# Iselix/kwiiyatta

Hardware: AMD Instinct MI355X
Metric: frames/sec end-to-end analyse->align->convert->synth, 48 kHz 5 ms hop (higher is better)
Workload: dtype f64; 1 GPU; config3: 48 kHz source (10 s, T=2001) + target (11 s, T=2201) pairs: CheapTrick+D4C of both, pad with freshly drawn silent spectra, sp2mc, FastDTW(radius 32) align, GMM(64 comp, D=144)+MLPG convert, mc2sp, WORLD synthesis; pairs_per_gpu=32, streams_per_gpu=4, GPU_MAX_HW_QUEUES=4, launch=the whole step is one captured HIP graph, gmm_model_prepared=once per converter (the per-mixture matrices depend on the GMM only), parallelism=pairs in lockstep x32 per GPU, pair-per-GPU x1, no collective

## Files before the change

### kwiiyatta_amd/csrc/kwy_d4c.hip

```cpp
#include <math.h>

#include <vector>

#include "kwy_internal.hpp"

#define D4C_SAFE 0.000000000001
#define D4C_FLOOR_F0 47.0
#define D4C_FREQ_INTERVAL 3000.0
#define D4C_UPPER_LIMIT 15000.0
#define D4C_MAX_BANDS 8

enum { D4C_HANNING = 1, D4C_BLACKMAN = 2 };

__device__ __forceinline__ double d4c_window(int type, int i, int half, double ratio, int fs, double cf0) {
  const double c1 = kwy_cos_pi_range(KWY_PI * ((2.0 * (i - half) / ratio) / fs) * cf0);
  return type == D4C_HANNING ? 0.5 * c1 + 0.5 : 0.42 + 0.5 * c1 + 0.08 * (2.0 * c1 * c1 - 1.0);
}

struct d4c_window_walk {
  double c, s, cd, sd;
  __device__ __forceinline__ d4c_window_walk(int i0, int step, int half, double ratio, int fs, double cf0) {
    kwy_sincos_pi_range(KWY_PI * ((2.0 * (i0 - half) / ratio) / fs) * cf0, &s, &c);
    sincos(KWY_PI * ((2.0 * step / ratio) / fs) * cf0, &sd, &cd);
  }
// ... 554 lines not shown
    constexpr int Q = (H / 2) / NT;
    static_assert(RK == 2 * Q + 1, "pairs per thread");
#pragma unroll
    for (int q = 0; q < Q; ++q)
      kwy_rfft_pair_power2_w<LOG2N - 1>(B, tid + NT * q, kwy_tw_hex(d4c_opaque(twb), HEX * q), &pv[2 * q], &pv[2 * q + 1]);
    pv[2 * Q] = 0.0;
    if (tid == 0) {
      double pm;
      kwy_rfft_pair_power2_w<LOG2N - 1>(B, H / 2, kwy_c{0.0, -1.0}, &pv[2 * Q], &pm);
    }
    __syncthreads();
#pragma unroll
    for (int q = 0; q < Q; ++q) {
      const int k = tid + NT * q;
      P[k] = pv[2 * q];
      P[H - k] = pv[2 * q + 1];
    }
    if (tid == 0) P[H / 2] = pv[2 * Q];
  }
  __syncthreads();
  d4c_dc_correction<NT>(P, S, cf0, p.fs, N);
  d4c_linear_smoothing_regs<NT, RK>(P, pv, S, tot, cf0, p.fs, N);

  D4C_STAMP(9);
#pragma unroll
  for (int r = 0; r < RP; ++r) {
    const int pp = DRAIN ? kwy_drain_bin<LOG2N - 1>(r, tid) : tid + NT * r;
    if (pp < H / 2) { Dv[pp] = cen_lo[r]; Dv[H - pp] = cen_hi[r]; }
  }
  if (tid == 0) Dv[H / 2] = mid[2];
  __syncthreads();
  d4c_dc_correction<NT>(Dv, S, cf0, p.fs, N);
#pragma unroll
  for (int r = 0; r < RK; ++r)
    if (tid + NT * r <= H) Dv[tid + NT * r] = Dv[tid + NT * r] / pv[r];
  __syncthreads();
  const int kdv = p.dv_len - 1;
  d4c_linear_smoothing<NT>(Dv, Dv, S, tot, cf0 / 2.0, p.fs, N, kdv + 2 * ((int)(cf0 * N / p.fs) + 1) + 4);
  d4c_subtract_smoothed<NT>(Dv, S, tot, cf0, p.fs, N, kdv);

  D4C_STAMP(10);
  {
    double *dv = dvbuf + (size_t)frame * p.dv_stride;
    for (int k = tid; k < p.dv_len; k += NT) dv[k] = Dv[k];
  }
  D4C_STAMP(15);
#undef D4C_STAMP
#undef D4C_BODY_TW4
}

template <int LOG2N>
static constexpr size_t d4c_bands_lds() {
  constexpr int N = 1 << LOG2N, H = N / 2, NT = d4c_nt<LOG2N>::value;
  return sizeof(double) * (16 + D4C_MAX_BANDS + 2 + 2 * NT) + sizeof(double) * ((2 * H + 2) + 2) +
         ((sizeof(uint32_t) * KWY_SELECT_WORDS(NT) > sizeof(double) * (2 * H + 4))
              ? sizeof(uint32_t) * KWY_SELECT_WORDS(NT) - sizeof(double) * (2 * H + 4) : 0);
}

template <int LOG2N, bool SPARSE>
__global__ __launch_bounds__(d4c_nt<LOG2N>::value, LOG2N >= 13 ? 2 : 4) void k_d4c_bands(
    d4c_batch batch, d4c_params p, const kwy_c *__restrict__ twH, const kwy_c *__restrict__ twP,
    const kwy_c *__restrict__ twN, const double *__restrict__ nuttall, long long *__restrict__ dbg) {
  constexpr int N = 1 << LOG2N, H = N / 2;
  constexpr int NT = d4c_nt<LOG2N>::value;
  constexpr int E = N / NT;
  constexpr int RK = (H + 1 + NT - 1) / NT;
  constexpr int HEX = 16 * NT / N;
  constexpr bool DRAIN = d4c_drain<LOG2N>::value;
#define D4C_STAMP(n) do { if (dbg && threadIdx.x == 0 && blockIdx.x == (unsigned)dbg[63]) dbg[n] = clock64(); } while (0)
  extern __shared__ double smem[];
  double *red = smem;
  double *coarse = red + 16;
  double *wns = coarse + D4C_MAX_BANDS + 2;
  kwy_c *B = (kwy_c *)(wns + 2 * NT);
  double *Bd = (double *)B;
  uint32_t *hist = (uint32_t *)B;

  const int tid = threadIdx.x;
  const int utt = batch.find(blockIdx.x);
  const int64_t frame = (int)blockIdx.x - batch.start[utt];
  const double *__restrict__ dvbuf = batch.u[utt].dvbuf;
  double *__restrict__ out = batch.u[utt].out;
  const double f0v = kwy_uniform(batch.u[utt].f0[frame]);
  if (f0v == 0.0 || kwy_uniform(batch.u[utt].ap0[frame]) <= p.threshold) return;
  const double cf0 = kwy_uniform(f0v > D4C_FLOOR_F0 ? f0v : D4C_FLOOR_F0);
  const double *Dv = dvbuf + (size_t)frame * p.dv_stride;
  D4C_STAMP(16);

  const int boundary = __builtin_amdgcn_readfirstlane(kwy_matlab_round(N * 8.0 / p.window_length));
  const int half_window_length = p.window_length / 2;
  constexpr bool sparse = SPARSE;
  double ns0 = 0.0, ns1 = 0.0, ns2 = 0.0, nutr[4] = {0.0, 0.0, 0.0, 0.0};
  if constexpr (sparse) {
    if (2 * tid < p.window_length) ns0 = nuttall[2 * tid];
    if (2 * tid + 1 < p.window_length) ns1 = nuttall[2 * tid + 1];
    wns[2 * tid] = ns0; wns[2 * tid + 1] = ns1;
  } else {
#pragma unroll
    for (int r = 0; r < 4; ++r)
      if (tid + NT * r < p.window_length) nutr[r] = nuttall[tid + NT * r];
  }
  const bool mine0 = sparse && tid < H / 8 && 2 * tid < p.window_length;
  const bool mine1 = sparse && tid < H / 8 && 2 * tid + 1 < p.window_length;
  const double *Dfirst = Dv + ((int)(D4C_FREQ_INTERVAL * N / p.fs) - half_window_length);
  double nx0 = (mine0 && p.nbands > 0) ? Dfirst[2 * tid] : 0.0;
  double nx1 = (mine1 && p.nbands > 0) ? Dfirst[2 * tid + 1] : 0.0;
  for (int b = 0; b < p.nbands; ++b) {
    const int tid = kwy_tid_opaque();
    kwy_c tw4[4];
    kwy_fft_thread_twiddles<LOG2N - 1, NT>(twH + (tid - (int)threadIdx.x), tw4);
    const kwy_c twb = twN[tid];
    const double *Dc = Dv + ((int)(D4C_FREQ_INTERVAL * (b + 1) * N / p.fs) - half_window_length);
    const double c0 = nx0, c1 = nx1;
    if (b == 1) D4C_STAMP(17);
    {
      const double *Dn = Dv + ((int)(D4C_FREQ_INTERVAL * (b + 2) * N / p.fs) - half_window_length);
      const bool more = b + 1 < p.nbands;
      nx0 = (mine0 && more) ? Dn[2 * tid] : 0.0;
      nx1 = (mine1 && more) ? Dn[2 * tid + 1] : 0.0;
    }
    if constexpr (sparse) {
      kwy_c a0 = {c0 * wns[2 * tid], c1 * wns[2 * tid + 1]}, a1 = {0.0, 0.0};
      if (tid == 0 && 2 * (H / 8) < p.window_length) a1.x = Dc[2 * (H / 8)] * nuttall[2 * (H / 8)];
      kwy_fft_pass8_first_sparse_core<LOG2N - 1, NT, false>(B, kwy_tw_reg{tw4[0]}, a0, a1);
      kwy_fft_inplace_rest_w<LOG2N - 1, NT, false, !DRAIN>(B, tw4, twP);
      if (b == 1) D4C_STAMP(18);
    } else {
#pragma unroll
      for (int r = 0; r < E; ++r) {
        const int j = tid + NT * r;
        Bd[j] = (r < 4 && j < p.window_length) ? Dc[j] * nutr[r < 4 ? r : 0] : 0.0;
      }
      __syncthreads();
      kwy_fft_inplace_w<LOG2N - 1, NT, false, !DRAIN>(B, tw4, twP);
    }
    unsigned long long key[RK];
    constexpr int Q = (H / 2) / NT;
    static_assert(RK == 2 * Q + 1, "pairs per thread");
    if constexpr (DRAIN) {
      static_assert(Q == 4 && sizeof(uint32_t) * KWY_SELECT_WORDS(NT) <= sizeof(kwy_c) * NT, "exchange clear of the histogram");
      kwy_c lo[4], hi[4], md;
      kwy_fft_tail4_drain<LOG2N - 1, NT, false>(B, lo, hi, md);
      const kwy_c twc = D4C_DRAIN_TWC(twN, NT, tid);
      double pw[8];
#pragma unroll
      for (int s = 0; s < 4; ++s) {
        if (s == 0 && tid == 0) kwy_rfft_pair_power2_dc(lo[0], &pw[0], &pw[1]);
        else kwy_rfft_pair_power2_v(lo[s], hi[s], kwy_drain_tw<LOG2N - 1, NT>(s, d4c_opaque(twb), twc), &pw[2 * s], &pw[2 * s + 1]);
      }
      key[2 * Q] = ~0ull;
      if (tid == 0) {
        double pk, pm;
        kwy_rfft_pair_power2_v(md, md, kwy_c{0.0, -1.0}, &pk, &pm);
        key[2 * Q] = (unsigned long long)__double_as_longlong(pk);
      } else {
        B[2 * NT - tid] = kwy_c{pw[4], pw[5]};
        B[4 * NT - tid] = kwy_c{pw[6], pw[7]};
      }
      __syncthreads();
      if (tid != 0) {
        const kwy_c v1 = B[NT + tid], v3 = B[3 * NT + tid];
        pw[4] = v1.x; pw[5] = v1.y; pw[6] = v3.x; pw[7] = v3.y;
      }
      key[0] = (unsigned long long)__double_as_longlong(pw[0]); key[1] = (unsigned long long)__double_as_longlong(pw[1]);
      key[2] = (unsigned long long)__double_as_longlong(pw[4]); key[3] = (unsigned long long)__double_as_longlong(pw[5]);
      key[4] = (unsigned long long)__double_as_longlong(pw[2]); key[5] = (unsigned long long)__double_as_longlong(pw[3]);
      key[6] = (unsigned long long)__double_as_longlong(pw[6]); key[7] = (unsigned long long)__double_as_longlong(pw[7]);
    } else {
#pragma unroll
      for (int q = 0; q < Q; ++q) {
        double pk, pm;
        kwy_rfft_pair_power2_w<LOG2N - 1>(B, tid + NT * q, kwy_tw_hex(d4c_opaque(twb), HEX * q), &pk, &pm);
        key[2 * q] = (unsigned long long)__double_as_longlong(pk);
        key[2 * q + 1] = (unsigned long long)__double_as_longlong(pm);
      }
      key[2 * Q] = ~0ull;
      if (tid == 0) {
        double pk, pm;
        kwy_rfft_pair_power2_w<LOG2N - 1>(B, H / 2, kwy_c{0.0, -1.0}, &pk, &pm);
        key[2 * Q] = (unsigned long long)__double_as_longlong(pk);
      }
      __syncthreads();
    }
    if (b == 1) D4C_STAMP(19);
    double nsmall, nall;
    kwy_block_smallest_sum<RK, NT>(key, H + 1, H - boundary, hist, red, &nsmall, &nall);
    if (b == 1) D4C_STAMP(20);
    if (dbg && tid == 0 && blockIdx.x == (unsigned)dbg[63])
      for (int q = 0; q < 12; ++q) dbg[24 + 12 * (b & 1) + q] = hist[2 * KWY_SELECT_BINS + q];
    if (tid == 0) {
      double cv = 10 * log10(nsmall / nall);
      cv = cv + (cf0 - 100) / 50.0;
      coarse[b + 1] = cv < 0.0 ? cv : 0.0;
    }
    __syncthreads();
  }
  D4C_STAMP(21);
  if (tid == 0) {
    coarse[0] = -60.0;
    coarse[p.nbands + 1] = -D4C_SAFE;
  }
  __syncthreads();
  double *o = out + frame * p.K;
  const int nn = p.nbands + 2;
  for (int k = tid; k < p.K; k += NT) {
    double xi = (double)k * p.fs / p.fft_size;
    int seg = min((int)(xi / D4C_FREQ_INTERVAL) + 1, p.nbands + 1);
    if (seg < 1) seg = 1;
    if (seg > nn - 1) seg = nn - 1;
    double xa = (seg - 1 <= p.nbands) ? (seg - 1) * D4C_FREQ_INTERVAL : p.fs / 2.0;
    double xb = (seg <= p.nbands) ? seg * D4C_FREQ_INTERVAL : p.fs / 2.0;
    double sfrac = (xi - xa) / (xb - xa);
    double v = coarse[seg - 1] + sfrac * (coarse[seg] - coarse[seg - 1]);
    o[k] = exp10(v / 20.0);
  }
  D4C_STAMP(22);
#undef D4C_STAMP
}

template <int LOG2N>
static int launch_lt(kwy_ctx *ctx, const d4c_batch &b, int fs) {
  constexpr int N = 1 << LOG2N, H = N / 2;
  const kwy_c *twH, *twN, *twP;
  const uint4 *poly;
  KWY_TRY(kwy_get_twiddles(ctx, LOG2N - 1, &twH));
  KWY_TRY(kwy_get_twiddle_powers(ctx, LOG2N - 1, &twP));
  KWY_TRY(kwy_get_twiddles(ctx, LOG2N, &twN));
  constexpr int NT = d4c_nt<LOG2N>::value;
  KWY_TRY(kwy_get_poly_multi(ctx, N / NT, NT, &poly));
  size_t lds = sizeof(kwy_c) * (H + 1) + sizeof(double) * 8 + sizeof(uint32_t) * KWY_EBASE_WORDS;
  KWY_HIP(hipFuncSetAttribute((const void *)k_d4c_lovetrain<LOG2N, NT>,
                              hipFuncAttributeMaxDynamicSharedMemorySize, (int)lds));
  KWY_PROF(ctx, "k_d4c_lovetrain", hipLaunchKernelGGL((k_d4c_lovetrain<LOG2N, NT>), dim3((unsigned)b.start[b.n]), dim3(NT), lds,
                     ctx->stream, b, fs, kwy_randn(ctx), poly, twH, twP, twN));
  KWY_HIP(hipGetLastError());
  return KWY_OK;
}

template <int LOG2N>
static int launch_body(kwy_ctx *ctx, const d4c_batch &b, const d4c_params &p, const double *nuttall) {
  constexpr int N = 1 << LOG2N, H = N / 2;
  const kwy_c *twH, *twN, *twP;
  const uint4 *poly;
  KWY_TRY(kwy_get_twiddles(ctx, LOG2N - 1, &twH));
  KWY_TRY(kwy_get_twiddle_powers(ctx, LOG2N - 1, &twP));
  KWY_TRY(kwy_get_twiddles(ctx, LOG2N, &twN));
  constexpr int NT = d4c_nt<LOG2N>::value;
  KWY_TRY(kwy_get_poly_multi(ctx, N / NT, NT, &poly));
// ... 198 lines not shown
```

### kwiiyatta_amd/csrc/kwy_device.hpp

```cpp
#pragma once

#include <hip/hip_runtime.h>
#include <stdint.h>

#define KWY_THREADS 256
#define KWY_WAVES (KWY_THREADS / 64)
#define KWY_PI 3.1415926535897932384

struct kwy_rng {
  uint32_t x, y, z, w;
};

__device__ __forceinline__ void kwy_rng_seed(kwy_rng &r) {
  r.x = 123456789u; r.y = 362436069u; r.z = 521288629u; r.w = 88675123u;
}

__device__ __forceinline__ uint32_t kwy_rng_step(kwy_rng &r) {
  uint32_t t = r.x ^ (r.x << 11);
  r.x = r.y; r.y = r.z; r.z = r.w;
  r.w = (r.w ^ (r.w >> 19)) ^ (t ^ (t >> 8));
  return r.w;
}

__device__ __forceinline__ uint32_t kwy_rng_randn_raw(kwy_rng &r) {
// ... 373 lines not shown
}

template <int NT, class F>
__device__ inline void kwy_block_count_scan(F count, int64_t n, uint64_t *__restrict__ offsets, uint64_t *tot) {
  const int t = threadIdx.x;
  const int64_t chunk = (n + NT - 1) / NT;
  const int64_t b0 = t * chunk, b1 = min(n, b0 + chunk);
  uint64_t run = 0;
  for (int64_t i = b0; i < b1; ++i) run += count(i);
  tot[t] = run;
  __syncthreads();
  if (t < 64) {
    constexpr int PER = NT / 64;
    uint64_t a[PER], acc = 0;
#pragma unroll
    for (int q = 0; q < PER; ++q) { a[q] = acc; acc += tot[PER * t + q]; }
    uint64_t inc = acc;
#pragma unroll
    for (int o = 1; o < 64; o <<= 1) {
      const uint64_t up = __shfl_up(inc, o);
      if (t >= o) inc += up;
    }
    const uint64_t excl = inc - acc;
#pragma unroll
    for (int q = 0; q < PER; ++q) tot[PER * t + q] = excl + a[q];
  }
  __syncthreads();
  run = tot[t];
  for (int64_t i = b0; i < b1; ++i) { offsets[i] = run; run += count(i); }
  if (b0 < n && b1 == n) offsets[n] = run;
  if (n == 0 && t == 0) offsets[0] = 0;
}

template <int NT = KWY_THREADS>
__device__ __forceinline__ void kwy_block_sum2(double a, double b, double *red, double *ta, double *tb) {
  a = kwy_wave_sum(a);
  b = kwy_wave_sum(b);
  __syncthreads();
  if ((threadIdx.x & 63) == 0) { red[threadIdx.x >> 6] = a; red[NT / 64 + (threadIdx.x >> 6)] = b; }
  __syncthreads();
  double sa = red[0], sb = red[NT / 64];
#pragma unroll
  for (int i = 1; i < NT / 64; ++i) { sa += red[i]; sb += red[NT / 64 + i]; }
  *ta = sa; *tb = sb;
}

#ifndef KWY_SELECT_BITS
#define KWY_SELECT_BITS 8
#endif
#define KWY_SELECT_BINS (1 << KWY_SELECT_BITS)
#ifndef KWY_SELECT_AGG
#define KWY_SELECT_AGG 0
#endif
#define KWY_SELECT_WORDS(NT) (2 * KWY_SELECT_BINS + 32)
#define KWY_SELECT_LIST (KWY_SELECT_BINS / 2 - 4)

__device__ __forceinline__ uint32_t kwy_wave_max_u32(uint32_t v) {
  v = max(v, (uint32_t)__builtin_amdgcn_update_dpp((int)v, (int)v, 0x101, 0xf, 0xf, false));
  v = max(v, (uint32_t)__builtin_amdgcn_update_dpp((int)v, (int)v, 0x102, 0xf, 0xf, false));
  v = max(v, (uint32_t)__builtin_amdgcn_update_dpp((int)v, (int)v, 0x104, 0xf, 0xf, false));
  v = max(v, (uint32_t)__builtin_amdgcn_update_dpp((int)v, (int)v, 0x108, 0xf, 0xf, false));
  return max(max((uint32_t)__builtin_amdgcn_readlane((int)v, 0), (uint32_t)__builtin_amdgcn_readlane((int)v, 16)),
             max((uint32_t)__builtin_amdgcn_readlane((int)v, 32), (uint32_t)__builtin_amdgcn_readlane((int)v, 48)));
}

__device__ __forceinline__ void kwy_select_scan(const uint32_t *h, int kk, uint32_t *ctl, int lane) {
  constexpr int PERLANE = KWY_SELECT_BINS / 64;
  static_assert(PERLANE % 4 == 0 && PERLANE >= 4, "bins per lane must be a multiple of 4");
  const uint4 *hp = (const uint4 *)h + lane * (PERLANE / 4);
  uint32_t tot = 0;
#pragma unroll
  for (int q = 0; q < PERLANE / 4; ++q) {
    const uint4 c4 = hp[q];
    tot += (c4.x + c4.y) + (c4.z + c4.w);
  }
  uint32_t before = kwy_wave_scan_u32(tot) - tot;
  if ((uint32_t)kk > before && (uint32_t)kk <= before + tot) {
    const uint32_t *hb = h + PERLANE * lane;
    for (int q = 0; q < PERLANE; ++q) {
      const uint32_t c = hb[q];
      if ((uint32_t)kk <= before + c) {
        ctl[0] = PERLANE * lane + q;
        ctl[1] = (uint32_t)kk - before;
        ctl[2] = c;
        ctl[3] = before;
        break;
      }
      before += c;
    }
  }
}

template <bool DESCENDING>
__device__ __forceinline__ void kwy_select_rank(const unsigned long long *list, int pop, int rank, int tid,
                                                unsigned long long *out_key, uint32_t *out_count) {
  if (tid < pop) {
    const unsigned long long mine = list[tid];
    int front = 0, tie_front = 0, ties = 0;
    for (int j = 0; j < pop; j += 4) {
      const ulonglong2 o01 = *(const ulonglong2 *)(list + j), o23 = *(const ulonglong2 *)(list + j + 2);
      const unsigned long long o[4] = {o01.x, o01.y, o23.x, o23.y};
#pragma unroll
      for (int q = 0; q < 4; ++q) {
        const bool in = j + q < pop;
        front += in & (DESCENDING ? o[q] > mine : o[q] < mine);
        const bool eq = in & (o[q] == mine);
        ties += eq;
        tie_front += eq & (j + q < tid);
      }
    }
    if (front + tie_front == rank - 1) { *out_key = mine; out_count[0] = (uint32_t)front; out_count[1] = (uint32_t)ties; }
  }
}

template <int RMAX, int NT = KWY_THREADS>
__device__ inline void kwy_block_smallest_sum(unsigned long long (&key)[RMAX], int n, int m,
                                              uint32_t *hist, double *red, double *sum_small,
                                              double *sum_all) {
  constexpr int BITS = KWY_SELECT_BITS, BINS = 1 << BITS;
  constexpr int TOP_SHIFT = 18;
  const int tid = threadIdx.x, lane = tid & 63, wv = tid >> 6;
  uint32_t *ctlb = hist + 2 * BINS;
  unsigned long long *k64 = (unsigned long long *)(ctlb + 8);
  unsigned long long *list = (unsigned long long *)(hist + BINS);
  unsigned long long vkey;
  int copies;

  uint32_t hmax = 0;
#pragma unroll
  for (int r = 0; r < RMAX; ++r)
    if (tid + NT * r < n) hmax = max(hmax, (uint32_t)(key[r] >> 32));
  hmax = kwy_wave_max_u32(hmax);
  if (lane == 0) ctlb[16 + wv] = hmax;
  for (int i = tid; i < BINS; i += NT) hist[i] = 0;
  if (tid == 0) ctlb[10] = 0;
  __syncthreads();
  hmax = ctlb[16];
#pragma unroll
  for (int i = 1; i < NT / 64; ++i) hmax = max(hmax, ctlb[16 + i]);
  uint32_t dg[RMAX];
#pragma unroll
  for (int r = 0; r < RMAX; ++r) {
    dg[r] = BINS;
    if (NT * r + (tid & ~63) >= n) continue;
    if (tid + NT * r < n) {
      dg[r] = min((hmax - (uint32_t)(key[r] >> 32)) >> TOP_SHIFT, (uint32_t)(BINS - 1));
      atomicAdd(&hist[dg[r]], 1u);
    }
  }
  __syncthreads();
  if (wv == 0) kwy_select_scan(hist, n - m + 1, ctlb, lane);
  __syncthreads();
  const uint32_t chosen = ctlb[0], pop = ctlb[2];
  if (chosen < (uint32_t)(BINS - 1) && pop <= (uint32_t)KWY_SELECT_LIST) {
    const int rank = (int)ctlb[1], above = (int)ctlb[3];
#pragma unroll
    for (int r = 0; r < RMAX; ++r)
      if (dg[r] == chosen) list[atomicAdd(&ctlb[10], 1u)] = key[r];
    __syncthreads();
    kwy_select_rank<true>(list, (int)pop, rank, tid, k64, &ctlb[11]);
    __syncthreads();
    vkey = *k64;
    copies = m - (n - above - (int)ctlb[11] - (int)ctlb[12]);
  } else {
    double lo = INFINITY, hi = 0.0;
#pragma unroll
    for (int r = 0; r < RMAX; ++r) {
      if (tid + NT * r < n) {
        const double x = __longlong_as_double((long long)key[r]);
        lo = fmin(lo, x); hi = fmax(hi, x);
      }
    }
    lo = kwy_wave_min_f64(lo);
    hi = kwy_wave_max_f64(hi);
    if (lane == 0) { red[wv] = lo; red[NT / 64 + wv] = hi; }
    for (int i = tid; i < BINS; i += NT) hist[i] = 0;
    if (tid == 0) ctlb[10] = 0;
    __syncthreads();
    lo = red[0]; hi = red[NT / 64];
#pragma unroll
    for (int i = 1; i < NT / 64; ++i) { lo = fmin(lo, red[i]); hi = fmax(hi, red[NT / 64 + i]); }
    const unsigned long long kmin = (unsigned long long)__double_as_longlong(lo);
    const unsigned long long range = (unsigned long long)__double_as_longlong(hi) - kmin;
    const int top0 = range ? 64 - __clzll((long long)range) : 0;
    const int rounds = (top0 + BITS - 1) / BITS;
#pragma unroll
    for (int r = 0; r < RMAX; ++r) key[r] -= kmin;
    unsigned long long prefix = 0ull;
    int kk = m;
    bool alive[RMAX];
#pragma unroll
    for (int r = 0; r < RMAX; ++r) alive[r] = tid + NT * r < n;
    for (int round = 0; round < rounds; ++round) {
      const int top = top0 - BITS * round;
      const int shift = top - BITS > 0 ? top - BITS : 0;
      const unsigned long long mask = (1ull << (top - shift)) - 1ull;
      uint32_t *h = hist + (round & 1) * BINS, *hn = hist + ((round + 1) & 1) * BINS;
      uint32_t *ctl = ctlb + (round & 1) * 4;
      for (int i = tid; i < BINS; i += NT) hn[i] = 0;
#pragma unroll
      for (int r = 0; r < RMAX; ++r) {
        if (NT * r + (tid & ~63) >= n) continue;
        const int d = (int)((key[r] >> shift) & mask);
#if KWY_SELECT_AGG
        const unsigned long long mm = __ballot(alive[r]);
        if (mm != 0ull) {
          const int leader = __builtin_amdgcn_readfirstlane(__ffsll((long long)mm) - 1);
          const int d0 = __builtin_amdgcn_readlane(d, leader);
          const bool same = alive[r] && d == d0;
          const unsigned long long ms = __ballot(same);
          if (lane == leader) atomicAdd(&h[d0], (uint32_t)__popcll(ms));
          if (alive[r] && !same) atomicAdd(&h[d], 1u);
        }
#else
        if (alive[r]) atomicAdd(&h[d], 1u);
#endif
      }
      __syncthreads();
      if (wv == 0) kwy_select_scan(h, kk, ctl, lane);
      __syncthreads();
      const int chosen_d = (int)ctl[0];
      prefix |= (unsigned long long)chosen_d << shift;
      kk = (int)ctl[1];
#pragma unroll
      for (int r = 0; r < RMAX; ++r) alive[r] = alive[r] && (int)((key[r] >> shift) & mask) == chosen_d;
      const uint32_t left = ctl[2];
      if (left == 1u && round < rounds - 1) {
#pragma unroll
        for (int r = 0; r < RMAX; ++r)
          if (alive[r]) *k64 = key[r];
        __syncthreads();
        prefix = *k64;
        kk = 1;
        break;
      }
      if (left <= (uint32_t)KWY_SELECT_LIST && round < rounds - 1) {
        unsigned long long *lst = (unsigned long long *)hn;
#pragma unroll
        for (int r = 0; r < RMAX; ++r)
          if (alive[r]) lst[atomicAdd(&ctlb[10], 1u)] = key[r];
        __syncthreads();
        kwy_select_rank<false>(lst, (int)left, kk, tid, k64, &ctlb[11]);
        __syncthreads();
        prefix = *k64;
        kk -= (int)ctlb[11];
        break;
      }
    }
    vkey = prefix + kmin;
    copies = kk;
#pragma unroll
    for (int r = 0; r < RMAX; ++r) key[r] += kmin;
  }
  const double vstar = __longlong_as_double((long long)vkey);
  double s_less = 0.0, s_all = 0.0;
#pragma unroll
  for (int r = 0; r < RMAX; ++r) {
    if (tid + NT * r < n) {
      const double x = __longlong_as_double((long long)key[r]);
      s_all += x;
      if (key[r] < vkey) s_less += x;
    }
  }
  double t_less, t_all;
  kwy_block_sum2<NT>(s_less, s_all, red, &t_less, &t_all);
  *sum_small = t_less + (double)copies * vstar;
  *sum_all = t_all;
}

struct __attribute__((aligned(16))) kwy_c { double x, y; };

__device__ __forceinline__ kwy_c cadd(kwy_c a, kwy_c b) { return {a.x + b.x, a.y + b.y}; }
__device__ __forceinline__ kwy_c csub(kwy_c a, kwy_c b) { return {a.x - b.x, a.y - b.y}; }
__device__ __forceinline__ kwy_c cmul(kwy_c a, kwy_c b) {
  return {a.x * b.x - a.y * b.y, a.x * b.y + a.y * b.x};
}
__device__ __forceinline__ kwy_c cmulf(kwy_c a, kwy_c b) {
  return {__builtin_fma(a.x, b.x, -(a.y * b.y)), __builtin_fma(a.x, b.y, a.y * b.x)};
}

__device__ __forceinline__ kwy_c kwy_tw_octant(kwy_c b, int r) {
  const double h = 0.70710678118654752440;
  switch (r & 7) {
    case 0: return b;
    case 1: return {h * (b.x + b.y), h * (b.y - b.x)};
    case 2: return {b.y, -b.x};
    case 3: return {h * (b.y - b.x), h * (-b.x - b.y)};
    case 4: return {-b.x, -b.y};
    case 5: return {h * (-b.x - b.y), h * (b.x - b.y)};
    case 6: return {-b.y, b.x};
    default: return {h * (b.x - b.y), h * (b.x + b.y)};
  }
}

template <bool INV>
__device__ __forceinline__ kwy_c kwy_rot90(kwy_c a) {
  return INV ? kwy_c{-a.y, a.x} : kwy_c{a.y, -a.x};
}

template <bool INV>
__device__ __forceinline__ void kwy_dft8(kwy_c (&a)[8]) {
  const double h = 0.70710678118654752440;
  kwy_c t0 = cadd(a[0], a[4]), t1 = csub(a[0], a[4]);
  kwy_c t2 = cadd(a[2], a[6]), t3 = kwy_rot90<INV>(csub(a[2], a[6]));
  kwy_c t4 = cadd(a[1], a[5]), t5 = csub(a[1], a[5]);
  kwy_c t6 = cadd(a[3], a[7]), t7 = csub(a[3], a[7]);
  kwy_c u0 = cadd(t0, t2), u1 = csub(t0, t2), u2 = cadd(t4, t6), u3 = kwy_rot90<INV>(csub(t4, t6));
  kwy_c c1 = INV ? kwy_c{h * (t5.x - t5.y), h * (t5.x + t5.y)} : kwy_c{h * (t5.x + t5.y), h * (t5.y - t5.x)};
  kwy_c c3 = INV ? kwy_c{h * (-t7.x - t7.y), h * (t7.x - t7.y)} : kwy_c{h * (t7.y - t7.x), h * (-t7.x - t7.y)};
  kwy_c v0 = cadd(t1, t3), v1 = csub(t1, t3), v2 = cadd(c1, c3), v3 = kwy_rot90<INV>(csub(c1, c3));
  a[0] = cadd(u0, u2); a[4] = csub(u0, u2); a[2] = cadd(u1, u3); a[6] = csub(u1, u3);
  a[1] = cadd(v0, v2); a[5] = csub(v0, v2); a[3] = cadd(v1, v3); a[7] = csub(v1, v3);
}

struct kwy_tw_table {
  const kwy_c *tw;
  __device__ __forceinline__ kwy_c operator()(int ps) const { return tw[ps]; }
};
#define KWY_TWP_ENTRY 8
#define KWY_TWP_ENTRIES(LOG2H) ((1 << (LOG2H)) / 512)
// ... 388 lines not shown
```

### kwiiyatta_amd/csrc/kwy_selftest.h

```cpp
#ifndef KWY_SELFTEST_H_
#define KWY_SELFTEST_H_
#ifdef __cplusplus
extern "C" {
#endif
int kwy_debug_smallest_sum_dev(void *stream, const double *values, int problems, int n, int m, double *out);
int kwy_debug_devmath_dev(void *stream, const double *x, int n, double *log_out, double *sin_out, double *cos_out);
int kwy_debug_rfft_paths_dev(void *stream, const double *x, int problems, int log2n, double *out_old, double *out_new);
int kwy_debug_fft_powers_dev(void *stream, const double *x, int problems, int log2h, int nt, int inverse,
                             double *out_lane, double *out_table, double *tab, double *tab_ref, double *tab_ref_conj);
#ifdef __cplusplus
}
#endif
#endif
```

### kwiiyatta_amd/csrc/selftest/kwy_selftest.hip

```cpp
#include <hip/hip_runtime.h>

#include <math.h>
#include <stdint.h>

#include <vector>

#include "../kwy_device.hpp"
#include "../kwy_selftest.h"

#define D4C_NT 256

__global__ __launch_bounds__(D4C_NT) void k_select_selftest(const double *__restrict__ v, int n, int m,
                                                           double *__restrict__ out) {
  constexpr int RK = 9;
  __shared__ __attribute__((aligned(16))) uint32_t hist[KWY_SELECT_WORDS(D4C_NT)];
  __shared__ double red[2 * D4C_NT / 64];
  const int tid = threadIdx.x;
  const double *x = v + (size_t)blockIdx.x * n;
  unsigned long long key[RK];
#pragma unroll
  for (int r = 0; r < RK; ++r) {
    const int k = tid + D4C_NT * r;
    key[r] = k < n ? (unsigned long long)__double_as_longlong(x[k]) : ~0ull;
  }
  double s_small, s_all;
  kwy_block_smallest_sum<RK, D4C_NT>(key, n, m, hist, red, &s_small, &s_all);
  if (tid == 0) { out[2 * blockIdx.x] = s_small; out[2 * blockIdx.x + 1] = s_all; }
}

extern "C" int kwy_debug_smallest_sum_dev(void *stream, const double *values, int problems, int n, int m,
                                          double *out) {
  if (!values || !out || problems <= 0 || n <= 0 || n > 9 * D4C_NT || m <= 0 || m > n) return -1;
  hipLaunchKernelGGL(k_select_selftest, dim3(problems), dim3(D4C_NT), 0, (hipStream_t)stream, values, n, m, out);
  return hipGetLastError() == hipSuccess ? 0 : -2;
}

__global__ void k_devmath_selftest(const double *__restrict__ x, int n, double *__restrict__ lg, double *__restrict__ sn,
                                   double *__restrict__ cs) {
  const int i = blockIdx.x * blockDim.x + threadIdx.x;
  if (i >= n) return;
  lg[i] = kwy_log(x[i]);
  kwy_sincos_medium(x[i], &sn[i], &cs[i]);
}

extern "C" int kwy_debug_devmath_dev(void *stream, const double *x, int n, double *log_out, double *sin_out,
                                     double *cos_out) {
  if (!x || !log_out || !sin_out || !cos_out || n <= 0) return -1;
  hipLaunchKernelGGL(k_devmath_selftest, dim3((n + 255) / 256), dim3(256), 0, (hipStream_t)stream, x, n, log_out,
                     sin_out, cos_out);
  return hipGetLastError() == hipSuccess ? 0 : -2;
}

template <int LOG2N, int NT>
__global__ __launch_bounds__(NT) void k_rfft_paths_selftest(const double *__restrict__ x, const kwy_c *__restrict__ twH,
                                                            const kwy_c *__restrict__ twP,
                                                            const kwy_c *__restrict__ twN, kwy_c *__restrict__ out_old,
                                                            kwy_c *__restrict__ out_new) {
  constexpr int N = 1 << LOG2N, H = N / 2, HEX = 16 * NT / N;
  extern __shared__ double smem[];
  kwy_c *B = (kwy_c *)smem;
  double *Bd = smem;
  const int tid = threadIdx.x;
  const double *row = x + (size_t)blockIdx.x * N;
  kwy_c *oo = out_old + (size_t)blockIdx.x * (H + 1), *on = out_new + (size_t)blockIdx.x * (H + 1);
  kwy_c tw4[4];
  kwy_fft_thread_twiddles<LOG2N - 1, NT>(twH, tw4);
  for (int i = tid; i < N; i += NT) Bd[i] = row[i];
  __syncthreads();
  kwy_fft_inplace_w<LOG2N - 1, NT, false>(B, tw4, twP);
  for (int r = 0; tid + NT * r <= H; ++r) {
    const int k = tid + NT * r;
    const kwy_c w = r < 4 ? kwy_tw_hex(twN[tid], HEX * r) : twN[k];
    oo[k] = kwy_rfft_bin2_w<LOG2N - 1>(B, k, w);
  }
  __syncthreads();
  for (int i = tid; i < N; i += NT) Bd[i] = row[i];
  __syncthreads();
  kwy_fft_inplace_w<LOG2N - 1, NT, false, false>(B, tw4, twP);
  kwy_c lo[4], hi[4], md;
  kwy_fft_tail4_drain<LOG2N - 1, NT, false>(B, lo, hi, md);
  const kwy_c twa = twN[tid], twc = twN[(NT - tid) & (NT - 1)];
#pragma unroll
  for (int s = 0; s < 4; ++s) {
    const int k = kwy_drain_bin<LOG2N - 1>(s, tid);
    if (k == 0) {
      on[0] = {2.0 * (lo[0].x + lo[0].y), 0.0};
// ... 121 lines not shown
```

Before: 2.774 million frames/s.

## Spread select histogram atomics over lane copies and trim block reductions in D4C

```diff
diff --git a/kwiiyatta_amd/csrc/kwy_d4c.hip b/kwiiyatta_amd/csrc/kwy_d4c.hip
--- a/kwiiyatta_amd/csrc/kwy_d4c.hip
+++ b/kwiiyatta_amd/csrc/kwy_d4c.hip
@@ -630,9 +630,9 @@
 template <int LOG2N>
 static constexpr size_t d4c_bands_lds() {
   constexpr int N = 1 << LOG2N, H = N / 2, NT = d4c_nt<LOG2N>::value;
+  constexpr size_t sel = sizeof(uint32_t) * (KWY_SELECT_WORDS(NT) + (d4c_drain<LOG2N>::value ? 0 : KWY_SELECT_WIDE_WORDS));
   return sizeof(double) * (16 + D4C_MAX_BANDS + 2 + 2 * NT) + sizeof(double) * ((2 * H + 2) + 2) +
-         ((sizeof(uint32_t) * KWY_SELECT_WORDS(NT) > sizeof(double) * (2 * H + 4))
-              ? sizeof(uint32_t) * KWY_SELECT_WORDS(NT) - sizeof(double) * (2 * H + 4) : 0);
+         (sel > sizeof(double) * (2 * H + 4) ? sel - sizeof(double) * (2 * H + 4) : 0);
 }
 
 template <int LOG2N, bool SPARSE>
@@ -653,6 +653,7 @@
   kwy_c *B = (kwy_c *)(wns + 2 * NT);
   double *Bd = (double *)B;
   uint32_t *hist = (uint32_t *)B;
+  uint32_t *wide = DRAIN ? (uint32_t *)(B + 4 * NT) : hist + KWY_SELECT_WORDS(NT);
 
   const int tid = threadIdx.x;
   const int utt = batch.find(blockIdx.x);
@@ -716,7 +717,9 @@
     constexpr int Q = (H / 2) / NT;
     static_assert(RK == 2 * Q + 1, "pairs per thread");
     if constexpr (DRAIN) {
-      static_assert(Q == 4 && sizeof(uint32_t) * KWY_SELECT_WORDS(NT) <= sizeof(kwy_c) * NT, "exchange clear of the histogram");
+      static_assert(Q == 4 && sizeof(uint32_t) * KWY_SELECT_WORDS(NT) <= sizeof(kwy_c) * NT &&
+                    sizeof(kwy_c) * 4 * NT + sizeof(uint32_t) * KWY_SELECT_WIDE_WORDS <= sizeof(kwy_c) * (H + 1),
+                    "exchange clear of the select's words");
       kwy_c lo[4], hi[4], md;
       kwy_fft_tail4_drain<LOG2N - 1, NT, false>(B, lo, hi, md);
       const kwy_c twc = D4C_DRAIN_TWC(twN, NT, tid);
@@ -762,16 +765,18 @@
     }
     if (b == 1) D4C_STAMP(19);
     double nsmall, nall;
-    kwy_block_smallest_sum<RK, NT>(key, H + 1, H - boundary, hist, red, &nsmall, &nall);
+    kwy_block_smallest_sum<RK, NT, false>(key, H + 1, H - boundary, hist, wide, red, &nsmall, &nall);
     if (b == 1) D4C_STAMP(20);
-    if (dbg && tid == 0 && blockIdx.x == (unsigned)dbg[63])
-      for (int q = 0; q < 12; ++q) dbg[24 + 12 * (b & 1) + q] = hist[2 * KWY_SELECT_BINS + q];
+    if (dbg) {
+      if (tid == 0 && blockIdx.x == (unsigned)dbg[63])
+        for (int q = 0; q < 12; ++q) dbg[24 + 12 * (b & 1) + q] = hist[2 * KWY_SELECT_BINS + q];
+      __syncthreads();
+    }
     if (tid == 0) {
       double cv = 10 * log10(nsmall / nall);
       cv = cv + (cf0 - 100) / 50.0;
       coarse[b + 1] = cv < 0.0 ? cv : 0.0;
     }
-    __syncthreads();
   }
   D4C_STAMP(21);
   if (tid == 0) {
diff --git a/kwiiyatta_amd/csrc/kwy_device.hpp b/kwiiyatta_amd/csrc/kwy_device.hpp
--- a/kwiiyatta_amd/csrc/kwy_device.hpp
+++ b/kwiiyatta_amd/csrc/kwy_device.hpp
@@ -449,7 +449,11 @@
 #ifndef KWY_SELECT_AGG
 #define KWY_SELECT_AGG 0
 #endif
-#define KWY_SELECT_WORDS(NT) (2 * KWY_SELECT_BINS + 32)
+#ifndef KWY_SELECT_COPIES
+#define KWY_SELECT_COPIES 4
+#endif
+#define KWY_SELECT_WORDS(NT) (2 * KWY_SELECT_BINS + 64)
+#define KWY_SELECT_WIDE_WORDS (KWY_SELECT_BINS * KWY_SELECT_COPIES)
 #define KWY_SELECT_LIST (KWY_SELECT_BINS / 2 - 4)
 
 __device__ __forceinline__ uint32_t kwy_wave_max_u32(uint32_t v) {
@@ -461,7 +465,7 @@
              max((uint32_t)__builtin_amdgcn_readlane((int)v, 32), (uint32_t)__builtin_amdgcn_readlane((int)v, 48)));
 }
 
-__device__ __forceinline__ void kwy_select_scan(const uint32_t *h, int kk, uint32_t *ctl, int lane) {
+__device__ __forceinline__ bool kwy_select_scan_lane(const uint32_t *h, int kk, int lane, uint32_t (&c)[4]) {
   constexpr int PERLANE = KWY_SELECT_BINS / 64;
   static_assert(PERLANE % 4 == 0 && PERLANE >= 4, "bins per lane must be a multiple of 4");
   const uint4 *hp = (const uint4 *)h + lane * (PERLANE / 4);
@@ -472,50 +476,68 @@
     tot += (c4.x + c4.y) + (c4.z + c4.w);
   }
   uint32_t before = kwy_wave_scan_u32(tot) - tot;
-  if ((uint32_t)kk > before && (uint32_t)kk <= before + tot) {
+  const bool mine = (uint32_t)kk > before && (uint32_t)kk <= before + tot;
+  c[0] = c[1] = c[2] = c[3] = 0u;
+  if (mine) {
     const uint32_t *hb = h + PERLANE * lane;
     for (int q = 0; q < PERLANE; ++q) {
-      const uint32_t c = hb[q];
-      if ((uint32_t)kk <= before + c) {
-        ctl[0] = PERLANE * lane + q;
-        ctl[1] = (uint32_t)kk - before;
-        ctl[2] = c;
-        ctl[3] = before;
+      const uint32_t n = hb[q];
+      if ((uint32_t)kk <= before + n) {
+        c[0] = PERLANE * lane + q;
+        c[1] = (uint32_t)kk - before;
+        c[2] = n;
+        c[3] = before;
         break;
       }
-      before += c;
-    }
-  }
-}
-
+      before += n;
+    }
+  }
+  return mine;
+}
+
+__device__ __forceinline__ void kwy_select_scan(const uint32_t *h, int kk, uint32_t *ctl, int lane) {
+  uint32_t c[4];
+  if (kwy_select_scan_lane(h, kk, lane, c)) { ctl[0] = c[0]; ctl[1] = c[1]; ctl[2] = c[2]; ctl[3] = c[3]; }
+}
+
+template <bool DESCENDING>
+__device__ __forceinline__ bool kwy_select_rank_entry(const unsigned long long *list, int pop, int rank, int e,
+                                                      unsigned long long mine, int *front_out, int *ties_out) {
+  int front = 0, tie_front = 0, ties = 0;
+  for (int j = 0; j < pop; j += 4) {
+    const ulonglong2 o01 = *(const ulonglong2 *)(list + j), o23 = *(const ulonglong2 *)(list + j + 2);
+    const unsigned long long o[4] = {o01.x, o01.y, o23.x, o23.y};
+#pragma unroll
+    for (int q = 0; q < 4; ++q) {
+      const bool in = j + q < pop;
+      front += in & (DESCENDING ? o[q] > mine : o[q] < mine);
+      const bool eq = in & (o[q] == mine);
+      ties += eq;
+      tie_front += eq & (j + q < e);
+    }
+  }
+  *front_out = front; *ties_out = ties;
+  return front + tie_front == rank - 1;
+}
 template <bool DESCENDING>
 __device__ __forceinline__ void kwy_select_rank(const unsigned long long *list, int pop, int rank, int tid,
                                                 unsigned long long *out_key, uint32_t *out_count) {
   if (tid < pop) {
     const unsigned long long mine = list[tid];
-    int front = 0, tie_front = 0, ties = 0;
-    for (int j = 0; j < pop; j += 4) {
-      const ulonglong2 o01 = *(const ulonglong2 *)(list + j), o23 = *(const ulonglong2 *)(list + j + 2);
-      const unsigned long long o[4] = {o01.x, o01.y, o23.x, o23.y};
-#pragma unroll
-      for (int q = 0; q < 4; ++q) {
-        const bool in = j + q < pop;
-        front += in & (DESCENDING ? o[q] > mine : o[q] < mine);
-        const bool eq = in & (o[q] == mine);
-        ties += eq;
-        tie_front += eq & (j + q < tid);
-      }
-    }
-    if (front + tie_front == rank - 1) { *out_key = mine; out_count[0] = (uint32_t)front; out_count[1] = (uint32_t)ties; }
-  }
-}
-
-template <int RMAX, int NT = KWY_THREADS>
+    int front, ties;
+    if (kwy_select_rank_entry<DESCENDING>(list, pop, rank, tid, mine, &front, &ties)) {
+      *out_key = mine; out_count[0] = (uint32_t)front; out_count[1] = (uint32_t)ties;
+    }
+  }
+}
+template <int RMAX, int NT = KWY_THREADS, bool ALL = true>
 __device__ inline void kwy_block_smallest_sum(unsigned long long (&key)[RMAX], int n, int m,
-                                              uint32_t *hist, double *red, double *sum_small,
+                                              uint32_t *hist, uint32_t *wide, double *red, double *sum_small,
                                               double *sum_all) {
-  constexpr int BITS = KWY_SELECT_BITS, BINS = 1 << BITS;
+  constexpr int BITS = KWY_SELECT_BITS, BINS = 1 << BITS, C = KWY_SELECT_COPIES;
   constexpr int TOP_SHIFT = 18;
+  static_assert(C == 1 || (C >= 4 && C <= 64 && (C & (C - 1)) == 0), "copies: one, or a power of two in whole 16-byte reads");
+  static_assert(NT <= 512, "the general path's extrema take 4 NT / 64 control words");
   const int tid = threadIdx.x, lane = tid & 63, wv = tid >> 6;
   uint32_t *ctlb = hist + 2 * BINS;
   unsigned long long *k64 = (unsigned long long *)(ctlb + 8);
@@ -524,12 +546,23 @@
   int copies;
 
   uint32_t hmax = 0;
-#pragma unroll
-  for (int r = 0; r < RMAX; ++r)
-    if (tid + NT * r < n) hmax = max(hmax, (uint32_t)(key[r] >> 32));
+  double s_all = 0.0;
+#pragma unroll
+  for (int r = 0; r < RMAX; ++r) {
+    if (tid + NT * r < n) {
+      hmax = max(hmax, (uint32_t)(key[r] >> 32));
+      s_all += __longlong_as_double((long long)key[r]);
+    }
+  }
   hmax = kwy_wave_max_u32(hmax);
-  if (lane == 0) ctlb[16 + wv] = hmax;
-  for (int i = tid; i < BINS; i += NT) hist[i] = 0;
+  s_all = kwy_wave_sum(s_all);
+  if (lane == 0) { ctlb[16 + wv] = hmax; red[NT / 64 + wv] = s_all; }
+  if constexpr (C > 1) {
+    static_assert(C == 1 || BINS * C % 4 == 0, "cleared in 16-byte stores");
+    for (int i = tid; i < BINS * C / 4; i += NT) ((uint4 *)wide)[i] = make_uint4(0u, 0u, 0u, 0u);
+  } else {
+    for (int i = tid; i < BINS; i += NT) hist[i] = 0;
+  }
   if (tid == 0) ctlb[10] = 0;
   __syncthreads();
   hmax = ctlb[16];
@@ -542,15 +575,29 @@
     if (NT * r + (tid & ~63) >= n) continue;
     if (tid + NT * r < n) {
       dg[r] = min((hmax - (uint32_t)(key[r] >> 32)) >> TOP_SHIFT, (uint32_t)(BINS - 1));
-      atomicAdd(&hist[dg[r]], 1u);
-    }
-  }
-  __syncthreads();
+      if constexpr (C > 1) atomicAdd(&wide[dg[r] * C + (lane & (C - 1))], 1u);
+      else atomicAdd(&hist[dg[r]], 1u);
+    }
+  }
+  __syncthreads();
+  if constexpr (C > 1) {
+    for (int b = tid; b < BINS; b += NT) {
+      const uint4 *bp = (const uint4 *)(wide + b * C);
+      uint32_t c = 0;
+#pragma unroll
+      for (int q = 0; q < C / 4; ++q) {
+        const uint4 c4 = bp[(q + b / (64 / C)) & (C / 4 - 1)];
+        c += (c4.x + c4.y) + (c4.z + c4.w);
+      }
+      hist[b] = c;
+    }
+    __syncthreads();
+  }
   if (wv == 0) kwy_select_scan(hist, n - m + 1, ctlb, lane);
   __syncthreads();
   const uint32_t chosen = ctlb[0], pop = ctlb[2];
+  const int rank = (int)ctlb[1], above = (int)ctlb[3];
   if (chosen < (uint32_t)(BINS - 1) && pop <= (uint32_t)KWY_SELECT_LIST) {
-    const int rank = (int)ctlb[1], above = (int)ctlb[3];
 #pragma unroll
     for (int r = 0; r < RMAX; ++r)
       if (dg[r] == chosen) list[atomicAdd(&ctlb[10], 1u)] = key[r];
@@ -558,8 +605,10 @@
     kwy_select_rank<true>(list, (int)pop, rank, tid, k64, &ctlb[11]);
     __syncthreads();
     vkey = *k64;
-    copies = m - (n - above - (int)ctlb[11] - (int)ctlb[12]);
+    const int front = (int)ctlb[11], ties = (int)ctlb[12];
+    copies = m - (n - above - front - ties);
   } else {
+    double *ext = (double *)(ctlb + 32);
     double lo = INFINITY, hi = 0.0;
 #pragma unroll
     for (int r = 0; r < RMAX; ++r) {
@@ -570,13 +619,13 @@
     }
     lo = kwy_wave_min_f64(lo);
     hi = kwy_wave_max_f64(hi);
-    if (lane == 0) { red[wv] = lo; red[NT / 64 + wv] = hi; }
+    if (lane == 0) { ext[wv] = lo; ext[NT / 64 + wv] = hi; }
     for (int i = tid; i < BINS; i += NT) hist[i] = 0;
     if (tid == 0) ctlb[10] = 0;
     __syncthreads();
-    lo = red[0]; hi = red[NT / 64];
-#pragma unroll
-    for (int i = 1; i < NT / 64; ++i) { lo = fmin(lo, red[i]); hi = fmax(hi, red[NT / 64 + i]); }
+    lo = ext[0]; hi = ext[NT / 64];
+#pragma unroll
+    for (int i = 1; i < NT / 64; ++i) { lo = fmin(lo, ext[i]); hi = fmax(hi, ext[NT / 64 + i]); }
     const unsigned long long kmin = (unsigned long long)__double_as_longlong(lo);
     const unsigned long long range = (unsigned long long)__double_as_longlong(hi) - kmin;
     const int top0 = range ? 64 - __clzll((long long)range) : 0;
@@ -650,19 +699,20 @@
     for (int r = 0; r < RMAX; ++r) key[r] += kmin;
   }
   const double vstar = __longlong_as_double((long long)vkey);
-  double s_less = 0.0, s_all = 0.0;
-#pragma unroll
-  for (int r = 0; r < RMAX; ++r) {
-    if (tid + NT * r < n) {
-      const double x = __longlong_as_double((long long)key[r]);
-      s_all += x;
-      if (key[r] < vkey) s_less += x;
-    }
-  }
-  double t_less, t_all;
-  kwy_block_sum2<NT>(s_less, s_all, red, &t_less, &t_all);
-  *sum_small = t_less + (double)copies * vstar;
-  *sum_all = t_all;
+  double s_less = 0.0;
+#pragma unroll
+  for (int r = 0; r < RMAX; ++r)
+    if (tid + NT * r < n && key[r] < vkey) s_less += __longlong_as_double((long long)key[r]);
+  s_less = kwy_wave_sum(s_less);
+  if (lane == 0) red[wv] = s_less;
+  __syncthreads();
+  if (ALL || tid == 0) {
+    double t_less = red[0], t_all = red[NT / 64];
+#pragma unroll
+    for (int i = 1; i < NT / 64; ++i) { t_less += red[i]; t_all += red[NT / 64 + i]; }
+    *sum_small = t_less + (double)copies * vstar;
+    *sum_all = t_all;
+  }
 }
 
 struct __attribute__((aligned(16))) kwy_c { double x, y; };
diff --git a/kwiiyatta_amd/csrc/kwy_selftest.h b/kwiiyatta_amd/csrc/kwy_selftest.h
--- a/kwiiyatta_amd/csrc/kwy_selftest.h
+++ b/kwiiyatta_amd/csrc/kwy_selftest.h
@@ -4,6 +4,10 @@
 extern "C" {
 #endif
 int kwy_debug_smallest_sum_dev(void *stream, const double *values, int problems, int n, int m, double *out);
+int kwy_debug_select_paths_dev(void *stream, const double *values, int problems, int n, int m, double *out_ref,
+                               double *out_new);
+int kwy_debug_select_paths512_dev(void *stream, const double *values, int problems, int n, int m, double *out_ref,
+                                  double *out_new);
 int kwy_debug_devmath_dev(void *stream, const double *x, int n, double *log_out, double *sin_out, double *cos_out);
 int kwy_debug_rfft_paths_dev(void *stream, const double *x, int problems, int log2n, double *out_old, double *out_new);
 int kwy_debug_fft_powers_dev(void *stream, const double *x, int problems, int log2h, int nt, int inverse,
diff --git a/kwiiyatta_amd/csrc/selftest/kwy_selftest.hip b/kwiiyatta_amd/csrc/selftest/kwy_selftest.hip
--- a/kwiiyatta_amd/csrc/selftest/kwy_selftest.hip
+++ b/kwiiyatta_amd/csrc/selftest/kwy_selftest.hip
@@ -13,7 +13,7 @@
 __global__ __launch_bounds__(D4C_NT) void k_select_selftest(const double *__restrict__ v, int n, int m,
                                                            double *__restrict__ out) {
   constexpr int RK = 9;
-  __shared__ __attribute__((aligned(16))) uint32_t hist[KWY_SELECT_WORDS(D4C_NT)];
+  __shared__ __attribute__((aligned(16))) uint32_t hist[KWY_SELECT_WORDS(D4C_NT) + KWY_SELECT_WIDE_WORDS];
   __shared__ double red[2 * D4C_NT / 64];
   const int tid = threadIdx.x;
   const double *x = v + (size_t)blockIdx.x * n;
@@ -24,7 +24,7 @@
     key[r] = k < n ? (unsigned long long)__double_as_longlong(x[k]) : ~0ull;
   }
   double s_small, s_all;
-  kwy_block_smallest_sum<RK, D4C_NT>(key, n, m, hist, red, &s_small, &s_all);
+  kwy_block_smallest_sum<RK, D4C_NT>(key, n, m, hist, hist + KWY_SELECT_WORDS(D4C_NT), red, &s_small, &s_all);
   if (tid == 0) { out[2 * blockIdx.x] = s_small; out[2 * blockIdx.x + 1] = s_all; }
 }
 
@@ -32,6 +32,201 @@
                                           double *out) {
   if (!values || !out || problems <= 0 || n <= 0 || n > 9 * D4C_NT || m <= 0 || m > n) return -1;
   hipLaunchKernelGGL(k_select_selftest, dim3(problems), dim3(D4C_NT), 0, (hipStream_t)stream, values, n, m, out);
+  return hipGetLastError() == hipSuccess ? 0 : -2;
+}
+
+#define REF_SELECT_WORDS (2 * KWY_SELECT_BINS + 32)
+template <int RMAX, int NT = KWY_THREADS>
+__device__ inline void ref_block_smallest_sum(unsigned long long (&key)[RMAX], int n, int m,
+                                              uint32_t *hist, double *red, double *sum_small,
+                                              double *sum_all) {
+  constexpr int BITS = KWY_SELECT_BITS, BINS = 1 << BITS;
+  constexpr int TOP_SHIFT = 18;
+  const int tid = threadIdx.x, lane = tid & 63, wv = tid >> 6;
+  uint32_t *ctlb = hist + 2 * BINS;
+  unsigned long long *k64 = (unsigned long long *)(ctlb + 8);
+  unsigned long long *list = (unsigned long long *)(hist + BINS);
+  unsigned long long vkey;
+  int copies;
+
+  uint32_t hmax = 0;
+#pragma unroll
+  for (int r = 0; r < RMAX; ++r)
+    if (tid + NT * r < n) hmax = max(hmax, (uint32_t)(key[r] >> 32));
+  hmax = kwy_wave_max_u32(hmax);
+  if (lane == 0) ctlb[16 + wv] = hmax;
+  for (int i = tid; i < BINS; i += NT) hist[i] = 0;
+  if (tid == 0) ctlb[10] = 0;
+  __syncthreads();
+  hmax = ctlb[16];
+#pragma unroll
+  for (int i = 1; i < NT / 64; ++i) hmax = max(hmax, ctlb[16 + i]);
+  uint32_t dg[RMAX];
+#pragma unroll
+  for (int r = 0; r < RMAX; ++r) {
+    dg[r] = BINS;
+    if (NT * r + (tid & ~63) >= n) continue;
+    if (tid + NT * r < n) {
+      dg[r] = min((hmax - (uint32_t)(key[r] >> 32)) >> TOP_SHIFT, (uint32_t)(BINS - 1));
+      atomicAdd(&hist[dg[r]], 1u);
+    }
+  }
+  __syncthreads();
+  if (wv == 0) kwy_select_scan(hist, n - m + 1, ctlb, lane);
+  __syncthreads();
+  const uint32_t chosen = ctlb[0], pop = ctlb[2];
+  if (chosen < (uint32_t)(BINS - 1) && pop <= (uint32_t)KWY_SELECT_LIST) {
+    const int rank = (int)ctlb[1], above = (int)ctlb[3];
+#pragma unroll
+    for (int r = 0; r < RMAX; ++r)
+      if (dg[r] == chosen) list[atomicAdd(&ctlb[10], 1u)] = key[r];
+    __syncthreads();
+    kwy_select_rank<true>(list, (int)pop, rank, tid, k64, &ctlb[11]);
+    __syncthreads();
+    vkey = *k64;
+    copies = m - (n - above - (int)ctlb[11] - (int)ctlb[12]);
+  } else {
+    double lo = INFINITY, hi = 0.0;
+#pragma unroll
+    for (int r = 0; r < RMAX; ++r) {
+      if (tid + NT * r < n) {
+        const double x = __longlong_as_double((long long)key[r]);
+        lo = fmin(lo, x); hi = fmax(hi, x);
+      }
+    }
+    lo = kwy_wave_min_f64(lo);
+    hi = kwy_wave_max_f64(hi);
+    if (lane == 0) { red[wv] = lo; red[NT / 64 + wv] = hi; }
+    for (int i = tid; i < BINS; i += NT) hist[i] = 0;
+    if (tid == 0) ctlb[10] = 0;
+    __syncthreads();
+    lo = red[0]; hi = red[NT / 64];
+#pragma unroll
+    for (int i = 1; i < NT / 64; ++i) { lo = fmin(lo, red[i]); hi = fmax(hi, red[NT / 64 + i]); }
+    const unsigned long long kmin = (unsigned long long)__double_as_longlong(lo);
+    const unsigned long long range = (unsigned long long)__double_as_longlong(hi) - kmin;
+    const int top0 = range ? 64 - __clzll((long long)range) : 0;
+    const int rounds = (top0 + BITS - 1) / BITS;
+#pragma unroll
+    for (int r = 0; r < RMAX; ++r) key[r] -= kmin;
+    unsigned long long prefix = 0ull;
+    int kk = m;
+    bool alive[RMAX];
+#pragma unroll
+    for (int r = 0; r < RMAX; ++r) alive[r] = tid + NT * r < n;
+    for (int round = 0; round < rounds; ++round) {
+      const int top = top0 - BITS * round;
+      const int shift = top - BITS > 0 ? top - BITS : 0;
+      const unsigned long long mask = (1ull << (top - shift)) - 1ull;
+      uint32_t *h = hist + (round & 1) * BINS, *hn = hist + ((round + 1) & 1) * BINS;
+      uint32_t *ctl = ctlb + (round & 1) * 4;
+      for (int i = tid; i < BINS; i += NT) hn[i] = 0;
+#pragma unroll
+      for (int r = 0; r < RMAX; ++r) {
+        if (NT * r + (tid & ~63) >= n) continue;
+        const int d = (int)((key[r] >> shift) & mask);
+#if KWY_SELECT_AGG
+        const unsigned long long mm = __ballot(alive[r]);
+        if (mm != 0ull) {
+          const int leader = __builtin_amdgcn_readfirstlane(__ffsll((long long)mm) - 1);
+          const int d0 = __builtin_amdgcn_readlane(d, leader);
+          const bool same = alive[r] && d == d0;
+          const unsigned long long ms = __ballot(same);
+          if (lane == leader) atomicAdd(&h[d0], (uint32_t)__popcll(ms));
+          if (alive[r] && !same) atomicAdd(&h[d], 1u);
+        }
+#else
+        if (alive[r]) atomicAdd(&h[d], 1u);
+#endif
+      }
+      __syncthreads();
+      if (wv == 0) kwy_select_scan(h, kk, ctl, lane);
+      __syncthreads();
+      const int chosen_d = (int)ctl[0];
+      prefix |= (unsigned long long)chosen_d << shift;
+      kk = (int)ctl[1];
+#pragma unroll
+      for (int r = 0; r < RMAX; ++r) alive[r] = alive[r] && (int)((key[r] >> shift) & mask) == chosen_d;
+      const uint32_t left = ctl[2];
+      if (left == 1u && round < rounds - 1) {
+#pragma unroll
+        for (int r = 0; r < RMAX; ++r)
+          if (alive[r]) *k64 = key[r];
+        __syncthreads();
+        prefix = *k64;
+        kk = 1;
+        break;
+      }
+      if (left <= (uint32_t)KWY_SELECT_LIST && round < rounds - 1) {
+        unsigned long long *lst = (unsigned long long *)hn;
+#pragma unroll
+        for (int r = 0; r < RMAX; ++r)
+          if (alive[r]) lst[atomicAdd(&ctlb[10], 1u)] = key[r];
+        __syncthreads();
+        kwy_select_rank<false>(lst, (int)left, kk, tid, k64, &ctlb[11]);
+        __syncthreads();
+        prefix = *k64;
+        kk -= (int)ctlb[11];
+        break;
+      }
+    }
+    vkey = prefix + kmin;
+    copies = kk;
+#pragma unroll
+    for (int r = 0; r < RMAX; ++r) key[r] += kmin;
+  }
+  const double vstar = __longlong_as_double((long long)vkey);
+  double s_less = 0.0, s_all = 0.0;
+#pragma unroll
+  for (int r = 0; r < RMAX; ++r) {
+    if (tid + NT * r < n) {
+      const double x = __longlong_as_double((long long)key[r]);
+      s_all += x;
+      if (key[r] < vkey) s_less += x;
+    }
+  }
+  double t_less, t_all;
+  kwy_block_sum2<NT>(s_less, s_all, red, &t_less, &t_all);
+  *sum_small = t_less + (double)copies * vstar;
+  *sum_all = t_all;
+}
+
+template <int NT>
+__global__ __launch_bounds__(NT) void k_select_paths_selftest(const double *__restrict__ v, int n, int m,
+                                                              double *__restrict__ out_ref, double *__restrict__ out_new) {
+  constexpr int RK = 9;
+  __shared__ __attribute__((aligned(16))) uint32_t hist[KWY_SELECT_WORDS(NT) + KWY_SELECT_WIDE_WORDS];
+  __shared__ double red[2 * NT / 64];
+  static_assert(REF_SELECT_WORDS <= KWY_SELECT_WORDS(NT), "the reference's scratch fits the current one's");
+  const int tid = threadIdx.x;
+  const double *x = v + (size_t)blockIdx.x * n;
+  unsigned long long key[RK];
+#pragma unroll
+  for (int r = 0; r < RK; ++r) {
+    const int k = tid + NT * r;
+    key[r] = k < n ? (unsigned long long)__double_as_longlong(x[k]) : ~0ull;
+  }
+  double s_small, s_all;
+  ref_block_smallest_sum<RK, NT>(key, n, m, hist, red, &s_small, &s_all);
+  if (tid == 0) { out_ref[2 * blockIdx.x] = s_small; out_ref[2 * blockIdx.x + 1] = s_all; }
+  __syncthreads();
+  kwy_block_smallest_sum<RK, NT, false>(key, n, m, hist, hist + KWY_SELECT_WORDS(NT), red, &s_small, &s_all);
+  if (tid == 0) { out_new[2 * blockIdx.x] = s_small; out_new[2 * blockIdx.x + 1] = s_all; }
+}
+
+extern "C" int kwy_debug_select_paths_dev(void *stream, const double *values, int problems, int n, int m,
+                                          double *out_ref, double *out_new) {
+  if (!values || !out_ref || !out_new || problems <= 0 || n <= 0 || n > 9 * 256 || m <= 0 || m > n) return -1;
+  hipLaunchKernelGGL(k_select_paths_selftest<256>, dim3(problems), dim3(256), 0, (hipStream_t)stream, values, n, m,
+                     out_ref, out_new);
+  return hipGetLastError() == hipSuccess ? 0 : -2;
+}
+
+extern "C" int kwy_debug_select_paths512_dev(void *stream, const double *values, int problems, int n, int m,
+                                             double *out_ref, double *out_new) {
+  if (!values || !out_ref || !out_new || problems <= 0 || n <= 0 || n > 9 * 512 || m <= 0 || m > n) return -1;
+  hipLaunchKernelGGL(k_select_paths_selftest<512>, dim3(problems), dim3(512), 0, (hipStream_t)stream, values, n, m,
+                     out_ref, out_new);
   return hipGetLastError() == hipSuccess ? 0 : -2;
 }
 
```

Result: faster. 2.811 million frames/s (median of 6 runs) (+1.3%).
